# arancormonk/dsd-neo

Hardware: AMD Instinct MI355X
Metric: I/Q Msamples/s end-to-end (demod->FEC->MBE) per GPU; % HBM roofline (higher is better)
Workload: dtype f32

## Files before the change

dsd-neo_amd/csrc/ddn_block.hip:

```cpp

#include <hip/hip_runtime.h>
#include <stdint.h>

#include <stdlib.h>
#include "ddn_device.h"
#include "ddn_nid_dev.h"

using namespace ddn_nid;

__global__ __launch_bounds__(64) void
k_nid_decode(const uint8_t* __restrict__ bits63, const uint8_t* __restrict__ rel63, const int32_t* __restrict__ obs_nac,
             const uint8_t* __restrict__ parity, const uint8_t* __restrict__ parity_rel, int threshold, int n,
             int32_t* __restrict__ out4, int32_t* __restrict__ chase_list, int32_t* __restrict__ chase_count) {
    __shared__ uint8_t ex[128];
    __shared__ uint8_t lg[64];
    __shared__ uint8_t work[(23 + 24 + 24 + 24) * 64];
    if (threadIdx.x == 0) {
        gf_fill(ex, lg);
    }
    __syncthreads();
    const Gf gf = {ex, lg};
    const Work wk = {work + threadIdx.x, work + 23 * 64 + threadIdx.x, work + 47 * 64 + threadIdx.x,
                     work + 71 * 64 + threadIdx.x};
    const int c = blockIdx.x * blockDim.x + threadIdx.x;
// ... 7 lines not shown
    }
    const int par = parity ? (parity[c] ? 1 : 0) : 0;
    const int prel = parity_rel ? parity_rel[c] : 0;
    const int obs = obs_nac ? obs_nac[c] : 0;
    const bool obs_ok = obs > 0 && obs < 0xFFF;

    int failed = 0;
    NidRes hard = nid_codeword(gf, wk, w, par, &failed);
    if (hard.status == 0 && failed && obs_ok && rx_nac(w) != obs) {
        hard = nid_codeword(gf, wk, put_nac(w, obs), par, nullptr);
    }
    NidRes res = hard;
    if (hard.status <= 0 && rel63 && chase_list) {
        chase_list[atomicAdd(chase_count, 1)] = c;
    } else if (hard.status <= 0 && rel63) {
        const uint8_t* rel = rel63 + (size_t)c * 63;
        uint64_t pool = 0;
        uint64_t taken = 0;
        int below = 0;
        for (int i = 0; i < 63; i++) {
            below += rel[i] < threshold;
        }
        for (int k = 0; k < 8; k++) {
            int bi = -1, bv = 256;
            for (int i = 0; i < 63; i++) {
                if (!((taken >> i) & 1) && rel[i] < bv) {
                    bv = rel[i];
                    bi = i;
                }
            }
            pool |= (uint64_t)bi << (8 * k);
            taken |= 1ull << bi;
        }
        int np = below < 8 ? below : 8;
        if (np < 6) {
            np = 6;
        }
        ChaseBest best = {0, {0, 0, 0, 0}, 0, 0};
        chase_from(gf, wk, w, rel, pool, np, par, prel, threshold, &best);
        if (obs_ok && rx_nac(w) != obs) {
            chase_from(gf, wk, put_nac(w, obs), rel, pool, np, par, prel, threshold, &best);
        }
        if (best.found) {
            res = best.dec;
        }
    }
    int32_t* o = out4 + (size_t)c * 4;
    o[0] = res.status;
    o[1] = res.nac;
    o[2] = res.duid;
    o[3] = res.errs;
}

__global__ void
k_hamming_10_6_3(uint8_t* __restrict__ bits10, int n, uint8_t* __restrict__ errs, DdnSel sel) {
    auto one = [&](long c) {
    uint8_t* b = bits10 + (size_t)c * 10;
    int word = 0;
    bool bad = false;
    for (int i = 0; i < 10; i++) {
        bad |= b[i] > 1;
        word = (word << 1) | (b[i] & 1);
    }
    if (bad) {
        errs[c] = 2;
        return;
    }
    const int masks[4] = {0x398, 0x354, 0x2E2, 0x1E1};
    int syn = 0;
    for (int k = 0; k < 4; k++) {
        syn = (syn << 1) | (__popc((unsigned)(word & masks[k])) & 1);
    }
    int e = 0;
    if (syn) {
        const int8_t bad_bit[16] = {-2, 0, 1, 5, 2, -1, -1, 6, 3, -1, -1, 7, 4, 8, 9, -1};
        const int bb = bad_bit[syn];
        if (bb < 0) {
            e = 2;
        } else {
            e = 1;
            if (bb >= 4) {
                word ^= 1 << bb;
            }
            for (int i = 0; i < 6; i++) {
                b[i] = (uint8_t)((word >> (9 - i)) & 1);
            }
        }
    }
    errs[c] = (uint8_t)e;
    };
    ddn_sel_for_each(sel, (long)n, one);
}

__global__ __launch_bounds__(64) void
k_nid_chase(const uint8_t* __restrict__ bits63, const uint8_t* __restrict__ rel63, const int32_t* __restrict__ obs_nac,
            const uint8_t* __restrict__ parity, const uint8_t* __restrict__ parity_rel, int threshold,
            const int32_t* __restrict__ chase_list, const int32_t* __restrict__ chase_count, int32_t* __restrict__ out4) {
    __shared__ uint8_t ex[128];
    __shared__ uint8_t lg[64];
    __shared__ uint8_t work[(23 + 24 + 24 + 24) * 64];
    __shared__ uint8_t masks[96];
    if ((int)blockIdx.x >= *chase_count) {
        return;
    }
    const int lane = threadIdx.x;
    if (lane == 0) {
        gf_fill(ex, lg);
// ... 170 lines not shown
            (void)hipFreeAsync(scratch, st);
        }
        return e;
    }
    hipLaunchKernelGGL(k_nid_chase, dim3((unsigned)n), dim3(64), 0, st, bits63, rel63, obs_nac, parity, parity_rel,
                       threshold, (const int32_t*)list, (const int32_t*)count, out4);
    e = hipGetLastError();
    const hipError_t ef = hipFreeAsync(scratch, st);
    return e != hipSuccess ? e : ef;
}

extern "C" hipError_t
ddn_dev_hamming_10_6_3(uint8_t* bits10, int n, uint8_t* errs, hipStream_t st) {
    if (n <= 0) {
        return hipSuccess;
    }
    const DdnSel sel = ddn_sel_for(24);
    hipLaunchKernelGGL(k_hamming_10_6_3, dim3(ddn_sel_grid(&sel, ((unsigned long)n + DDN_WG - 1) / DDN_WG)), dim3(DDN_WG), 0, st, bits10, n, errs, sel);
    return hipGetLastError();
}

namespace {
__device__ __forceinline__ int
lsd_parity_of(int data) {
    int v = data << 8;
#pragma unroll
    for (int i = 15; i >= 8; i--) {
        if (v & (1 << i)) {
            v ^= 0x139 << (i - 8);
        }
    }
    return v & 0xFF;
}

__device__ __forceinline__ int
lsd_hard(int word) {
    const int data = (word >> 8) & 0xFF, parity = word & 0xFF;
    const int synd = parity ^ lsd_parity_of(data);
    if (synd == 0) {
        return word;
    }
    if ((synd & (synd - 1)) == 0) {
        return word ^ synd;
    }
#pragma unroll
    for (int pos = 0; pos < 8; pos++) {
        if (lsd_parity_of(1 << (7 - pos)) == synd) {
            return word ^ (1 << (15 - pos));
        }
    }
    return -1;
}

__global__ void
k_p25_lsd(uint8_t* __restrict__ bits16, const int16_t* __restrict__ llr16, int n, uint8_t* __restrict__ ok, DdnSel sel) {
    auto one = [&](long i) {
    uint8_t* b = bits16 + (size_t)i * 16;
    int word = 0;
    for (int k = 0; k < 16; k++) {
        word = (word << 1) | (b[k] & 1);
    }
    int fixed = lsd_hard(word);
    if (fixed < 0 && llr16) {
        const int16_t* l = llr16 + (size_t)i * 16;
        int cand[6], rel[6], nc = 0;
        unsigned taken = 0;
        for (int c = 0; c < 6; c++) {
            int bi = -1, br = 1 << 30;
            for (int k = 0; k < 16; k++) {
                const int r = l[k] < 0 ? -(int)l[k] : (int)l[k];
                if (r < 64 && !(taken & (1u << k)) && r < br) {
                    br = r;
                    bi = k;
                }
            }
            if (bi < 0) {
                break;
            }
            taken |= 1u << bi;
            cand[nc] = bi;
            rel[nc] = br;
            nc++;
        }
        int best = -1, best_pen = 999999;
        for (int mask = 1; mask < (1 << nc); mask++) {
            int w = word, pen = 0;
            for (int c = 0; c < nc; c++) {
                if (mask & (1 << c)) {
                    w ^= 1 << (15 - cand[c]);
                    pen += rel[c];
                }
            }
            if (pen >= best_pen) {
                continue;
            }
            const int f = lsd_hard(w);
            if (f >= 0) {
                best = f;
                best_pen = pen;
            }
        }
        fixed = best;
    }
    if (fixed >= 0) {
        for (int k = 0; k < 16; k++) {
            b[k] = (uint8_t)((fixed >> (15 - k)) & 1);
        }
    }
    ok[i] = fixed >= 0 ? 1 : 0;
    };
    ddn_sel_for_each(sel, (long)n, one);
}
}

extern "C" hipError_t
ddn_dev_p25_lsd(uint8_t* bits16, const int16_t* llr16, int n, uint8_t* ok, hipStream_t st) {
    if (n <= 0) {
        return hipSuccess;
    }
    const DdnSel sel = ddn_sel_for(2);
    hipLaunchKernelGGL(k_p25_lsd, dim3(ddn_sel_grid(&sel, ((unsigned long)n + DDN_WG - 1) / DDN_WG)), dim3(DDN_WG), 0, st, bits16, llr16, n, ok, sel);
    return hipGetLastError();
}

namespace {
__global__ void
k_p25_crc16(const uint8_t* __restrict__ bytes, int item_bytes, int n, uint8_t* __restrict__ ok) {
    const int i = blockIdx.x * blockDim.x + threadIdx.x;
    if (i >= n) {
        return;
    }
    const uint8_t* b = bytes + (size_t)i * item_bytes;
    unsigned crc = 0;
    for (int k = 0; k < item_bytes - 2; k++) {
        const unsigned v = b[k];
#pragma unroll
        for (int j = 7; j >= 0; j--) {
            const unsigned bit = (v >> j) & 1u;
            crc = (((crc >> 15) & 1u) ^ bit) ? (((crc << 1) ^ 0x1021u) & 0xFFFFu) : ((crc << 1) & 0xFFFFu);
        }
    }
    crc ^= 0xFFFFu;
    ok[i] = crc == (((unsigned)b[item_bytes - 2] << 8) | b[item_bytes - 1]) ? 1 : 0;
// ... 12 lines not shown
```

dsd-neo_amd/csrc/ddn_mbe.hip:

```cpp

#include <hip/hip_runtime.h>
#include <mutex>
#include <stdint.h>

#include "ddn_device.h"
#include "ddn_mbe.h"
#include "ddn_mbe_dev.h"
#include "ddn_mbe_math.h"

namespace {

__device__ __forceinline__ uint32_t
golay_syndrome(uint32_t w) {
#pragma unroll
    for (int i = 22; i >= 11; i--) {
        if ((w >> i) & 1u) {
            w ^= 0xC75u << (i - 11);
        }
    }
    return w & 0x7FFu;
}

__device__ __forceinline__ void
golay_table_lds(uint32_t* tab, int tid, int nthreads) {
// ... 1 lines not shown
        const int a = idx / 529, b = (idx / 23) % 23, c = idx % 23;
        if (a <= b && b <= c) {
            const uint32_t e = (1u << a) | (1u << b) | (1u << c);
            tab[golay_syndrome(e)] = e;
        }
    }
    if (tid == 0) {
        tab[0] = 0;
    }
}

__device__ uint32_t g_golay_tab[2048];

__global__ __launch_bounds__(256) void
k_golay_tab_init() {
    __shared__ uint32_t tab[2048];
    for (int i = threadIdx.x; i < 2048; i += 256) {
        tab[i] = 0;
    }
    __syncthreads();
    golay_table_lds(tab, threadIdx.x, 256);
    __syncthreads();
    for (int i = threadIdx.x; i < 2048; i += 256) {
        g_golay_tab[i] = tab[i];
    }
}

__device__ __forceinline__ uint32_t
golay_fix(uint32_t w, const uint32_t* tab, int& errs) {
    const uint32_t e = tab[golay_syndrome(w)] & 0x7FF800u;
    errs = __popc(e);
    return w ^ e;
}

__device__ __forceinline__ uint32_t
hamming_fix(uint32_t w, int& errs) {
    const uint32_t m0 = 0x7f08, m1 = 0x78e4, m2 = 0x66d2, m3 = 0x55b1;
    const uint32_t syn = ((__popc(w & m0) & 1) << 3) | ((__popc(w & m1) & 1) << 2) | ((__popc(w & m2) & 1) << 1)
                         | (__popc(w & m3) & 1);
    errs = 0;
    if (syn) {
        errs = 1;
#pragma unroll
        for (int p = 0; p < 15; p++) {
            const uint32_t col = (((m0 >> p) & 1u) << 3) | (((m1 >> p) & 1u) << 2) | (((m2 >> p) & 1u) << 1) | ((m3 >> p) & 1u);
            if (col == syn) {
                w ^= 1u << p;
            }
        }
    }
    return w;
}

#define DDN_MBE_FRAMES_PER_WG 32
template <int CODEC>
__global__ __launch_bounds__(64) void
k_mbe_frame_decode(const uint8_t* __restrict__ frames, const uint8_t* __restrict__ soft, size_t n,
                   uint8_t* __restrict__ bits_out, int32_t* __restrict__ result) {
    constexpr int FB = CODEC == DDN_MBE_IMBE_7200X4400 ? 184 : 96;
    constexpr int OB = CODEC == DDN_MBE_IMBE_7200X4400 ? 88 : 49;
    constexpr int ROWLEN = CODEC == DDN_MBE_IMBE_7200X4400 ? 23 : 24;
    constexpr int FPW = DDN_MBE_FRAMES_PER_WG;
    __shared__ uint8_t stage[FPW * FB];
    __shared__ uint8_t outb[FPW * OB];
    const uint32_t* tab = g_golay_tab;
    const int lane = threadIdx.x;
    const size_t f0 = (size_t)blockIdx.x * FPW;
    const size_t nf = (n - f0) < (size_t)FPW ? (n - f0) : (size_t)FPW;
    const uint8_t* src = frames + f0 * FB;
    for (size_t i = lane; i < nf * FB; i += 64) {
        stage[i] = src[i];
    }
    __syncthreads();
    if ((size_t)lane < nf) {
        const uint8_t* f = stage + lane * FB;
        uint32_t row[8];
        bool bad = false;
        constexpr int NROW = CODEC == DDN_MBE_IMBE_7200X4400 ? 8 : 4;
#pragma unroll
        for (int r = 0; r < NROW; r++) {
            uint32_t w = 0;
            for (int j = 0; j < ROWLEN; j++) {
                const uint32_t v = f[r * ROWLEN + j];
                bad |= v > 1u;
                w |= (v & 1u) << j;
            }
            row[r] = w;
        }
        uint8_t* o = outb + lane * OB;
        int c0 = 0, c4 = 0, total = 0, e = 0;
        unsigned flags = MBE_PROCESS_FLAG_C0_VALID | (soft ? MBE_PROCESS_FLAG_SOFT_INPUT : 0u);
        if (CODEC == DDN_MBE_IMBE_7200X4400) {
            flags |= MBE_PROCESS_FLAG_C4_VALID;
            row[0] = golay_fix(row[0], tab, c0);
            total = c0;
            uint32_t pr = (16u * (row[0] >> 11)) & 0xFFFFu;
#pragma unroll
            for (int r = 1; r < 7; r++) {
                const int len = r < 4 ? 23 : 15;
                uint32_t mask = 0;
                for (int j = len - 1; j >= 0; j--) {
                    pr = (173u * pr + 13849u) & 0xFFFFu;
                    mask |= (pr >> 15) << j;
                }
                row[r] ^= mask;
            }
#pragma unroll
            for (int r = 1; r < 4; r++) {
                row[r] = golay_fix(row[r], tab, e);
                total += e;
            }
#pragma unroll
            for (int r = 4; r < 7; r++) {
                row[r] = hamming_fix(row[r] & 0x7FFFu, e);
                if (r == 4) {
                    c4 = e;
                }
                total += e;
            }
            int k = 0;
#pragma unroll
            for (int r = 0; r < 4; r++) {
                for (int j = 22; j > 10; j--) {
                    o[k++] = (uint8_t)((row[r] >> j) & 1u);
                }
            }
#pragma unroll
            for (int r = 4; r < 7; r++) {
                for (int j = 14; j >= 4; j--) {
                    o[k++] = (uint8_t)((row[r] >> j) & 1u);
                }
            }
            for (int j = 6; j >= 0; j--) {
                o[k++] = (uint8_t)((row[7] >> j) & 1u);
            }
        } else {
            uint32_t w0 = golay_fix(row[0] >> 1, tab, c0);
            row[0] = (w0 << 1) | (row[0] & 1u);
            uint32_t pr = (16u * (w0 >> 11)) & 0xFFFFu;
            uint32_t mask = 0;
            for (int j = 22; j >= 0; j--) {
                pr = (173u * pr + 13849u) & 0xFFFFu;
                mask |= (pr >> 15) << j;
            }
            row[1] = golay_fix((row[1] ^ mask) & 0x7FFFFFu, tab, e);
            total = c0 + e;
            int k = 0;
            for (int j = 23; j > 11; j--) {
                o[k++] = (uint8_t)((row[0] >> j) & 1u);
            }
            for (int j = 22; j > 10; j--) {
                o[k++] = (uint8_t)((row[1] >> j) & 1u);
            }
            for (int j = 10; j >= 0; j--) {
                o[k++] = (uint8_t)((row[2] >> j) & 1u);
            }
            for (int j = 13; j >= 0; j--) {
                o[k++] = (uint8_t)((row[3] >> j) & 1u);
            }
        }
        int32_t* r5 = result + (f0 + lane) * 5;
        if (bad) {
            for (int k = 0; k < OB; k++) {
                o[k] = 0;
            }
            r5[0] = (int32_t)DDN_MBE_RESULT_INVALID;
            r5[1] = r5[2] = r5[3] = r5[4] = 0;
        } else {
            r5[0] = (int32_t)flags;
            r5[1] = c0;
            r5[2] = c4;
            r5[3] = total;
            r5[4] = total - c0;
        }
    }
    __syncthreads();
    uint8_t* dst = bits_out + f0 * OB;
    for (size_t i = lane; i < nf * OB; i += 64) {
        dst[i] = outb[i];
    }
}

struct LaneParms {
    float w0, gamma;
    int L, K, repeat;
    int V;
    float Ml, log2Ml, PHI, PSI;
};

__device__ __forceinline__ LaneParms
lane_init(int l) {
    LaneParms p;
    p.w0 = 0.09378f;
    p.gamma = 0.0f;
    p.L = 30;
    p.K = 10;
    p.repeat = 0;
    p.V = 0;
    p.Ml = 0.0f;
    p.log2Ml = 0.0f;
    p.PHI = 0.0f;
    p.PSI = MBE_PI_F / 2.0f;
    (void)l;
    return p;
}

__device__ __forceinline__ LaneParms
lane_load(const mbe_parms* s, int l) {
    LaneParms p;
    const int i = l <= 56 ? l : 56;
    p.w0 = s->w0;
    p.gamma = s->gamma;
    p.L = s->L;
    p.K = s->K;
    p.repeat = s->repeat;
    p.V = s->Vl[i];
    p.Ml = s->Ml[i];
    p.log2Ml = s->log2Ml[i];
    p.PHI = s->PHIl[i];
    p.PSI = s->PSIl[i];
    return p;
}

__device__ __forceinline__ void
lane_store(mbe_parms* s, const LaneParms& p, int l, int un) {
    if (l == 0) {
        s->w0 = p.w0;
        s->gamma = p.gamma;
        s->L = p.L;
        s->K = p.K;
        s->repeat = p.repeat;
        s->un = un;
    }
    if (l <= 56) {
        s->Vl[l] = p.V;
        s->Ml[l] = p.Ml;
        s->log2Ml[l] = p.log2Ml;
        s->PHIl[l] = p.PHI;
        s->PSIl[l] = p.PSI;
    }
}

__device__ __forceinline__ float
dequant(uint32_t b, int bits, float step) {
    if (bits <= 0) {
        return 0.0f;
    }
    return step * (((float)b - (float)(1u << (bits - 1))) + 0.5f);
}

__device__ __forceinline__ float
idct_term(const float* C, int J, int j) {
    float acc = 0.0f;
    for (int k = 1; k <= J; k++) {
        const float a = (k == 1) ? 1.0f : 2.0f;
        const float ang = (MBE_PI_F * (float)(k - 1) * ((float)j - 0.5f)) / (float)J;
        acc = acc + (a * C[k]) * mbe_cosf(ang);
    }
    return acc;
}

template <int CODEC>
__global__ __launch_bounds__(64) void
k_mbe_params(const uint8_t* __restrict__ bits, const int32_t* __restrict__ res_in, int n_frames,
             const ddn_mbe_tables* __restrict__ T, const float* __restrict__ half_log2, DdnMbeStream* __restrict__ streams,
             int tail_rule, DdnMbeFrameRec* __restrict__ recs, int32_t* __restrict__ res_out) {
    constexpr int NB = CODEC == DDN_MBE_IMBE_7200X4400 ? 88 : 49;
    __shared__ uint32_t fld[64];
    __shared__ float sG[12], sR[12], sC[64], sPl[64], sA[64], sB[64];
    __shared__ float sCb[5][64];
    const int s = blockIdx.x;
    const int l = threadIdx.x;
    DdnMbeStream* st = streams + s;
    LaneParms cur = lane_load(&st->cur, l), prev = lane_load(&st->prev, l), enh = lane_load(&st->enh, l);
    uint32_t frame_no = st->frame_no;
    const uint32_t seed = st->seed;

    for (int f = 0; f < n_frames; f++) {
        const size_t fi = (size_t)s * (size_t)n_frames + (size_t)f;
        const uint8_t* d = bits + fi * NB;
        int32_t r[5] = {0, 0, 0, 0, 0};
        if (res_in) {
#pragma unroll
            for (int k = 0; k < 5; k++) {
                r[k] = res_in[fi * 5 + k];
            }
        }
        unsigned flags = (unsigned)r[0];
        const int errs2 = r[3];
        DdnMbeFrameRec* rec = recs + fi;
        const uint32_t v0 = (l < NB) ? d[l] : 0u, v1 = (l + 64 < NB) ? d[l + 64] : 0u;
        const unsigned long long m0 = __ballot(v0 & 1u), m1 = __ballot(v1 & 1u);
        const bool invalid = __any((v0 > 1u) || (v1 > 1u)) || (flags & DDN_MBE_RESULT_INVALID);
        auto bit = [&](int p) -> uint32_t { return (uint32_t)(((p < 64 ? m0 >> p : m1 >> (p - 64))) & 1ull); };
        bool skip = invalid;
        if (!skip && tail_rule && CODEC == DDN_MBE_IMBE_7200X4400 && errs2 >= 10) {
            uint32_t prefix = 0;
            for (int p = 0; p < 8; p++) {
                prefix = (prefix << 1) | bit(p);
            }
            const int set = __popcll(m0) + __popcll(m1 & 0xFFFFFFull);
            if (prefix == 0xFCu && set <= 24) {
                skip = true;
                flags = 0;
                r[1] = r[2] = r[3] = r[4] = 0;
            }
        }
        if (skip) {
            if (l == 0) {
                rec->flags = DDN_MBE_REC_SILENCE;
                rec->maxl = 0;
                if (res_out) {
                    res_out[fi * 5 + 0] = (int32_t)(invalid ? DDN_MBE_RESULT_INVALID : flags);
                    res_out[fi * 5 + 1] = r[1];
                    res_out[fi * 5 + 2] = r[2];
                    res_out[fi * 5 + 3] = r[3];
                    res_out[fi * 5 + 4] = r[4];
                }
            }
            continue;
        }

        cur.repeat = prev.repeat;
        int bad = 0;
        float Tl = 0.0f;
        float rho = 0.65f, extra = 0.0f;
        int L = 0;
        float unvc = 1.0f;
        if (CODEC == DDN_MBE_IMBE_7200X4400) {
            uint32_t b0 = 0;
            for (int p = 0; p < 6; p++) {
// ... 131 lines not shown
                    sG[l] = T->ambe_prba24[b3][l - 2];
                } else if (l >= 5 && l <= 8) {
                    sG[l] = T->ambe_prba58[b4][l - 5];
                }
                __syncthreads();
                if (l >= 1 && l <= 8) {
                    sR[l] = idct_term(sG, 8, l);
                }
                __syncthreads();
                for (int i = 1; i <= 4; i++) {
                    sCb[i][l] = 0.0f;
                }
                __syncthreads();
                if (l < 24) {
                    const int i = l / 6 + 1, k = l % 6 + 1;
                    const int J = T->ambe_blocks[L][i - 1];
                    float c = 0.0f;
                    if (k == 1) {
                        c = 0.5f * (sR[2 * i - 1] + sR[2 * i]);
                    } else if (k == 2) {
                        c = 0.353553390593274f * (sR[2 * i - 1] - sR[2 * i]);
                    } else if (k <= J) {
                        const float* h = (i == 1) ? T->ambe_hoc5[b5] : ((i == 2) ? T->ambe_hoc6[b6] : ((i == 3) ? T->ambe_hoc7[b7] : T->ambe_hoc8[b8]));
                        c = h[k - 3];
                    }
                    sCb[i][k] = c;
                }
                __syncthreads();
                if (l >= 1 && l <= L) {
                    int first = 1, bi = 1, J = 1;
                    for (int i = 1; i <= 4; i++) {
                        J = T->ambe_blocks[L][i - 1];
                        bi = i;
                        if (l < first + J) {
                            break;
                        }
                        first += J;
                    }
                    Tl = idct_term(sCb[bi], J, l - first + 1);
                }
                sA[l] = Tl;
                __syncthreads();
                float tsum = 0.0f;
                for (int k = 1; k <= L; k++) {
                    tsum = tsum + sA[k];
                }
                extra = (cur.gamma - half_log2[L]) - (tsum / (float)L);
                rho = 0.65f;
                __syncthreads();
            }
        }
        if (bad == 0) {
            const int pL = prev.L;
            const float pl_edge = __shfl(prev.log2Ml, pL <= 56 ? pL : 56);
            const float pl_one = __shfl(prev.log2Ml, 1);
            sPl[l] = (l == 0) ? pl_one : ((l <= pL && l <= 56) ? prev.log2Ml : pl_edge);
            __syncthreads();
            const float ratio = (float)pL / (float)L;
            float sum = 0.0f;
            for (int k = 1; k <= L; k++) {
                const float kl = ratio * (float)k;
                const int ki = (int)kl;
                const float dl = kl - (float)ki;
                sum = sum + (((1.0f - dl) * sPl[ki]) + (dl * sPl[ki + 1]));
            }
            sum = sum * (rho / (float)L);
            if (l >= 1 && l <= L) {
                const float kl = ratio * (float)l;
                const int ki = (int)kl;
                const float dl = kl - (float)ki;
                cur.log2Ml = (((Tl + ((rho * (1.0f - dl)) * sPl[ki])) + ((rho * dl) * sPl[ki + 1])) - sum) + extra;
                const float m = mbe_expf(0.693f * cur.log2Ml);
                cur.Ml = (CODEC == DDN_MBE_AMBE_3600X2450 && !cur.V) ? unvc * m : m;
            }
            __syncthreads();
        }
        bool use_last;
        if (CODEC == DDN_MBE_IMBE_7200X4400) {
            use_last = (bad == 1) || (errs2 > 5);
        } else {
            use_last = (bad == 0) && (errs2 > 3);
        }
        if (use_last) {
            const int rp = cur.repeat;
            cur = prev;
            cur.repeat = rp + 1;
            flags |= MBE_PROCESS_FLAG_REPEAT;
        } else {
            cur.repeat = 0;
        }
        if ((CODEC == DDN_MBE_IMBE_7200X4400 || bad == 0) && cur.repeat <= 3) {
            prev = cur;
            const int cL = cur.L;
            const float cw = mbe_cosf(cur.w0 * (float)l);
            const float m2 = cur.Ml * cur.Ml;
            sA[l] = m2;
            sB[l] = m2 * cw;
            __syncthreads();
            float Rm0 = 0.0f, Rm1 = 0.0f;
            for (int k = 1; k <= cL; k++) {
                Rm0 = Rm0 + sA[k];
                Rm1 = Rm1 + sB[k];
            }
            __syncthreads();
            const float R2m0 = Rm0 * Rm0, R2m1 = Rm1 * Rm1;
            if (l >= 1 && l <= cL && cur.Ml != 0.0f) {
                const float num = (0.96f * MBE_PI_F) * ((R2m0 + R2m1) - (((2.0f * Rm0) * Rm1) * cw));
                const float den = (cur.w0 * Rm0) * (R2m0 - R2m1);
                const float x = num / den;
                float W = 1.0f;
                if (!((8 * l) <= cL || !(x > 0.0f) || !(x < 3.0e38f))) {
                    const float tmp = sqrtf(cur.Ml) * sqrtf(sqrtf(x));
                    W = (tmp > 1.2f) ? 1.2f : ((tmp < 0.5f) ? 0.5f : tmp);
                }
                cur.Ml = cur.Ml * W;
            }
            sA[l] = cur.Ml * cur.Ml;
            __syncthreads();
            float sum2 = 0.0f;
            for (int k = 1; k <= cL; k++) {
                sum2 = sum2 + sA[k];
            }
            __syncthreads();
            const float gam = (sum2 == 0.0f) ? 1.0f : sqrtf(Rm0 / sum2);
            if (l >= 1 && l <= cL) {
                cur.Ml = gam * cur.Ml;
            }
            const int num_uv = __popcll(__ballot(l >= 1 && l <= cL && cur.V == 0));
            const float cw0 = cur.w0, pw0 = enh.w0;
            int maxl;
            if (cL > enh.L) {
                maxl = cL;
                if (l > enh.L && l <= maxl) {
                    enh.Ml = 0.0f;
                    enh.V = 1;
                }
            } else {
                maxl = enh.L;
                if (l > cL && l <= maxl) {
                    cur.Ml = 0.0f;
                    cur.V = 1;
                }
            }
            const uint32_t fbase = mbe_mix(mbe_mix(0x9E3779B9u, seed), frame_no);
            if (l >= 1 && l <= 56) {
                float psi = enh.PSI + ((pw0 + cw0) * ((float)(l * 160) / 2.0f));
                psi = __builtin_fmaf(-__builtin_rintf(psi * 0.159154943091895336f), MBE_TWO_PI_F, psi);
                cur.PSI = psi;
                if (l <= (cL / 4)) {
                    cur.PHI = psi;
                } else {
                    cur.PHI = psi + (((float)num_uv * mbe_rand_phase(mbe_mix(mbe_mix(fbase, (uint32_t)l), 0x100u))) / (float)cL);
                }
            }
            const unsigned long long cvm = __ballot(cur.V != 0), pvm = __ballot(enh.V != 0);
            rec->cMl[l] = cur.Ml;
            rec->pMl[l] = enh.Ml;
            rec->cPHI[l] = cur.PHI;
            rec->pPHI[l] = enh.PHI;
            if (l == 0) {
                rec->cw0 = cw0;
                rec->pw0 = pw0;
                rec->maxl = maxl;
                rec->flags = 0;
                rec->cv_lo = (uint32_t)cvm;
                rec->cv_hi = (uint32_t)(cvm >> 32);
                rec->pv_lo = (uint32_t)pvm;
                rec->pv_hi = (uint32_t)(pvm >> 32);
                rec->fbase = fbase;
            }
            enh = cur;
        } else {
            flags |= MBE_PROCESS_FLAG_MUTE;
            cur = prev = enh = lane_init(l);
            if (l == 0) {
                rec->flags = DDN_MBE_REC_SILENCE;
                rec->maxl = 0;
            }
        }
        frame_no++;
        if (l == 0 && res_out) {
            res_out[fi * 5 + 0] = (int32_t)flags;
            res_out[fi * 5 + 1] = r[1];
            res_out[fi * 5 + 2] = r[2];
            res_out[fi * 5 + 3] = r[3];
            res_out[fi * 5 + 4] = r[4];
        }
    }
    lane_store(&st->cur, cur, l, (int)frame_no);
    lane_store(&st->prev, prev, l, (int)frame_no);
    lane_store(&st->enh, enh, l, (int)frame_no);
    if (l == 0) {
        st->frame_no = frame_no;
    }
}

__device__ __forceinline__ float
unvoiced_mix(float w0, float w0l, int l, int n, uint32_t base, uint32_t tag) {
    float c3 = 0.0f;
#pragma unroll
    for (int i = 0; i < 3; i++) {
        const float rph = mbe_rand_phase(mbe_mix(base, tag + (uint32_t)i));
        c3 = c3 + mbe_cosf(((w0 * (float)n) * (((float)l + ((float)i * MBE_UVSTEP)) - MBE_UVOFFSET)) + rph);
        if (w0l > MBE_UVTHRESHOLD) {
            c3 = c3 + (((w0l - MBE_UVTHRESHOLD) * MBE_UVRAND) * mbe_u01(mbe_mix(mbe_mix(base, tag + 0x40u + (uint32_t)i), (uint32_t)n)));
        }
    }
    return c3;
}

__global__ __launch_bounds__(64) void
k_mbe_synth(const DdnMbeFrameRec* __restrict__ recs, float* __restrict__ pcm) {
    const DdnMbeFrameRec* rec = recs + blockIdx.x;
    float* out = pcm + (size_t)blockIdx.x * 160;
    const int lane = threadIdx.x;
    const int maxl = rec->maxl;
    float acc[3] = {0.0f, 0.0f, 0.0f};
    if (!(rec->flags & DDN_MBE_REC_SILENCE)) {
        const float cw0 = rec->cw0, pw0 = rec->pw0;
        const uint32_t fbase = rec->fbase;
        const unsigned long long cvm = ((unsigned long long)rec->cv_hi << 32) | rec->cv_lo;
        const unsigned long long pvm = ((unsigned long long)rec->pv_hi << 32) | rec->pv_lo;
        const int nA = lane, nB = 56 + lane, nC = 105 + lane;
        const bool inA = lane < 56, inB = lane < 49, inC = lane < 55;
        const float wpA = mbe_ws(nA + 160), wpB = mbe_ws(nB + 160), wcB = mbe_ws(nB), wcC = mbe_ws(nC);
        for (int l = 1; l <= maxl; l++) {
            const float cw0l = cw0 * (float)l, pw0l = pw0 * (float)l;
            const uint32_t base = mbe_mix(fbase, (uint32_t)l);
            const int cv = (int)((cvm >> l) & 1ull), pv = (int)((pvm >> l) & 1ull);
            const float cM = rec->cMl[l], pM = rec->pMl[l], cP = rec->cPHI[l], pP = rec->pPHI[l];
            auto prev_side = [&](int n, float w) {
                if (pv == 1) {
                    return (w * pM) * mbe_cosf((pw0l * (float)n) + pP);
                }
                const float c3 = unvoiced_mix(pw0, pw0l, l, n, base, 0x300u);
                return (((c3 * MBE_UVSINE) * w) * pM) * MBE_QFACTOR;
            };
            auto cur_side = [&](int n, float w) {
                if (cv == 1) {
                    return (w * cM) * mbe_cosf((cw0l * (float)(n - 160)) + cP);
                }
                const float c3 = unvoiced_mix(cw0, cw0l, l, n, base, 0x200u);
                return (((c3 * MBE_UVSINE) * w) * cM) * MBE_QFACTOR;
// ... 132 lines not shown
```

dsd-neo_amd/csrc/ddn_rs.hip:

```cpp

#include <hip/hip_runtime.h>

#include <mutex>
#include <stdint.h>

#include "ddn_device.h"
#include "ddn_tables_isch.h"

namespace {
__device__ __forceinline__ uint32_t
golay_syndrome11(uint32_t cw) {
    cw &= 0x7fffffu;
#pragma unroll
    for (int i = 0; i < 12; i++) {
        cw = (cw & 1u) ? ((cw ^ 0xAE3u) >> 1) : (cw >> 1);
    }
    return cw;
}
}

__global__ void
k_golay_table(uint32_t* __restrict__ tab) {
    const int idx = blockIdx.x * blockDim.x + threadIdx.x;
    if (idx == 0) {
// ... 14 lines not shown
    auto one = [&](long i) {
    uint8_t* d = data + (size_t)i * len;
    const uint8_t* p = parity + (size_t)i * 12;
    uint32_t cw = 0;
    bool valid = true;
    for (int k = 0; k < 12; k++) {
        const uint32_t v = p[k];
        valid &= v <= 1;
        cw |= (v & 1u) << (12 + k);
    }
    for (int k = 0; k < len; k++) {
        const uint32_t v = d[k];
        valid &= v <= 1;
        cw |= (v & 1u) << (12 - len + k);
    }
    int fx = 0, rc = 1;
    if (valid) {
        const uint32_t pbit = cw & 0x800000u;
        uint32_t w23 = cw & 0x7fffffu;
        const uint32_t e = tab[golay_syndrome11(w23)];
        if (e) {
            const int wt = __popc(e);
            bool fits = false;
            uint32_t r = e;
#pragma unroll
            for (int k = 0; k < 23; k++) {
                fits |= (r & 0xFFFu) == 0;
                r = ((r << 1) | (r >> 22)) & 0x7fffffu;
            }
            fx = fits ? wt : wt - 1;
            w23 ^= e;
        }
        cw = w23 | pbit;
        const bool odd = (__popc(cw) & 1) != 0;
        if (!(odd && (cw & 0x3fu) != 0)) {
            rc = 0;
            for (int k = 0; k < len; k++) {
                d[k] = (uint8_t)((cw >> (12 - len + k)) & 1u);
            }
        }
    }
    status[i] = (uint8_t)rc;
    if (fixed) {
        fixed[i] = fx;
    }
    };
    ddn_sel_for_each(sel, (long)n, one);
}

__global__ __launch_bounds__(64) void
k_rs63(uint8_t* __restrict__ data6, const uint8_t* __restrict__ parity6, int n_par, int n_data, int t, int n,
       uint8_t* __restrict__ status, DdnSel sel) {
    __shared__ uint8_t ex[128], lg[64];
    __shared__ uint8_t W[36][64];
    __shared__ uint8_t S[17][64], Cc[18][64], Bb[18][64], Tt[18][64], Om[16][64], Pos[8][64];
    const int lane = threadIdx.x;
    if (lane == 0) {
        int x = 1;
        for (int i = 0; i < 63; i++) {
            ex[i] = (uint8_t)x;
            ex[i + 63] = (uint8_t)x;
            lg[x] = (uint8_t)i;
            x <<= 1;
            if (x & 0x40) {
                x ^= 0x43;
            }
        }
        ex[126] = ex[0];
        ex[127] = ex[1];
        lg[0] = 0;
    }
    __syncthreads();
    auto one = [&](long i) {
    auto gmul = [&](int a, int b) -> int { return (a && b) ? ex[lg[a] + lg[b]] : 0; };
    auto gdiv = [&](int a, int b) -> int { return a ? ex[lg[a] + 63 - lg[b]] : 0; };
    auto gpow = [&](int a, int e) -> int { return a ? ex[(lg[a] + e) % 63] : 0; };
    const int nsym = n_par + n_data, n2 = 2 * t;
    uint8_t* dp = data6 + (size_t)i * n_data * 6;
    const uint8_t* pp = parity6 + (size_t)i * n_par * 6;
    for (int k = 0; k < nsym; k++) {
        const uint8_t* q = (k < n_par) ? (pp + 6 * k) : (dp + 6 * (k - n_par));
        int v = 0;
#pragma unroll
        for (int b = 0; b < 6; b++) {
            v = (v << 1) | (q[b] != 0);
        }
        W[k][lane] = (uint8_t)v;
    }
    int any = 0;
    for (int s = 1; s <= n2; s++) {
        int acc = 0;
        for (int j = 0; j < nsym; j++) {
            acc ^= gpow(W[j][lane], (s * j) % 63);
        }
        S[s][lane] = (uint8_t)acc;
        any |= acc;
    }
    int rc = 0;
    if (any) {
        for (int k = 0; k < 18; k++) {
            Cc[k][lane] = (k == 0);
            Bb[k][lane] = (k == 0);
        }
        int L = 0, m = 1, b = 1;
        for (int it = 0; it < n2; it++) {
            int d = S[it + 1][lane];
            for (int k = 1; k <= L; k++) {
                d ^= gmul(Cc[k][lane], S[it + 1 - k][lane]);
            }
            if (d == 0) {
                m++;
            } else {
                const int f = gdiv(d, b);
                const bool grow = 2 * L <= it;
                for (int k = 0; k < 18; k++) {
                    Tt[k][lane] = Cc[k][lane];
                }
                for (int k = 0; k + m < 18; k++) {
                    Cc[k + m][lane] ^= (uint8_t)gmul(f, Bb[k][lane]);
                }
                if (grow) {
                    L = it + 1 - L;
                    for (int k = 0; k < 18; k++) {
                        Bb[k][lane] = Tt[k][lane];
                    }
                    b = d;
                    m = 1;
                } else {
                    m++;
                }
            }
        }
        int deg = 0;
        for (int k = 17; k >= 0; k--) {
            if (Cc[k][lane]) {
                deg = k;
                break;
            }
        }
        if (L > t || deg != L) {
            rc = 1;
        } else {
            int np = 0;
            for (int p = 0; p < 63; p++) {
                const int xi = (63 - p) % 63;
                int v = 0;
                for (int k = 0; k <= L; k++) {
                    v ^= gpow(Cc[k][lane], (k * xi) % 63);
                }
                if (v == 0) {
                    if (np < 8) {
                        Pos[np][lane] = (uint8_t)p;
                    }
                    np++;
                }
            }
            if (np != L) {
                rc = 1;
            } else {
                for (int k = 0; k < n2; k++) {
                    int v = 0;
                    for (int j = 0; j <= k && j <= L; j++) {
                        v ^= gmul(Cc[j][lane], S[k - j + 1][lane]);
                    }
                    Om[k][lane] = (uint8_t)v;
                }
                int ev[8];
                for (int k = 0; k < 8; k++) {
                    ev[k] = 0;
                }
                for (int e = 0; e < L && rc == 0; e++) {
                    const int p = Pos[e][lane];
                    const int xi = (63 - p) % 63;
                    int num = 0, den = 0;
                    for (int k = 0; k < n2; k++) {
                        num ^= gpow(Om[k][lane], (k * xi) % 63);
                    }
                    for (int k = 1; k <= L; k += 2) {
                        den ^= gpow(Cc[k][lane], ((k - 1) * xi) % 63);
                    }
                    if (den == 0) {
                        rc = 1;
                    } else {
                        const int val = gdiv(num, den);
#pragma unroll
                        for (int k = 0; k < 8; k++) {
                            ev[k] = (k == e) ? val : ev[k];
                        }
                    }
                }
                if (rc == 0) {
#pragma unroll
                    for (int e = 0; e < 8; e++) {
                        if (e < L) {
                            const int p = Pos[e][lane];
                            if (p < nsym) {
                                W[p][lane] ^= (uint8_t)ev[e];
                            }
                        }
                    }
                    for (int k = 0; k < n_data; k++) {
                        const int v = W[n_par + k][lane];
#pragma unroll
                        for (int b = 0; b < 6; b++) {
                            dp[6 * k + b] = (uint8_t)((v >> (5 - b)) & 1);
                        }
                    }
                }
            }
        }
    } else {
        for (int k = 0; k < n_data; k++) {
            const int v = W[n_par + k][lane];
#pragma unroll
            for (int b = 0; b < 6; b++) {
                dp[6 * k + b] = (uint8_t)((v >> (5 - b)) & 1);
            }
        }
    }
    if (rc != 0) {
        for (int k = 0; k < n_data; k++) {
            const int v = W[n_par + k][lane];
#pragma unroll
            for (int b = 0; b < 6; b++) {
                dp[6 * k + b] = (uint8_t)((v >> (5 - b)) & 1);
            }
        }
    }
    status[i] = (uint8_t)rc;
    };
    ddn_sel_for_each(sel, (long)n, one);
}

__global__ __launch_bounds__(64) void
k_rs63_soft(uint8_t* __restrict__ data6, const uint8_t* __restrict__ parity6, const uint8_t* __restrict__ data_rel,
            const uint8_t* __restrict__ parity_rel, int n_par, int n_data, int t, int threshold, int n,
            uint8_t* __restrict__ status) {
    __shared__ uint8_t ex[128], lg[64];
    __shared__ uint8_t W[36][64], S[17][64], G[18][64], M[17][64], Cc[18][64], Bb[18][64], Tt[18][64], Lam[18][64],
        Om[16][64], Loc[16][64], Val[16][64], Er[16][64];
    __shared__ uint16_t Key[36][64];
    const int lane = threadIdx.x;
    if (lane == 0) {
        int x = 1;
        for (int i = 0; i < 63; i++) {
            ex[i] = (uint8_t)x;
            ex[i + 63] = (uint8_t)x;
            lg[x] = (uint8_t)i;
            x <<= 1;
            if (x & 0x40) {
                x ^= 0x43;
            }
        }
        ex[126] = ex[0];
        ex[127] = ex[1];
        lg[0] = 0;
    }
    __syncthreads();
    const int i = blockIdx.x * 64 + lane;
    if (i >= n) {
        return;
    }
    auto gmul = [&](int a, int b) -> int { return (a && b) ? ex[lg[a] + lg[b]] : 0; };
    auto gdiv = [&](int a, int b) -> int { return a ? ex[lg[a] + 63 - lg[b]] : 0; };
    auto gpow = [&](int a, int e) -> int { return a ? ex[(lg[a] + e) % 63] : 0; };
    const int nsym = n_par + n_data, n2 = 2 * t;
    uint8_t* dp = data6 + (size_t)i * n_data * 6;
    const uint8_t* pp = parity6 + (size_t)i * n_par * 6;
    for (int k = 0; k < nsym; k++) {
        const uint8_t* q = (k < n_par) ? (pp + 6 * k) : (dp + 6 * (k - n_par));
        int v = 0;
#pragma unroll
        for (int b = 0; b < 6; b++) {
            v = (v << 1) | (q[b] != 0);
        }
        W[k][lane] = (uint8_t)v;
    }
    int any = 0;
    for (int s = 1; s <= n2; s++) {
        int acc = 0;
// ... 1329 lines not shown
```

Baseline: 25300.

## Bit-pack MBE frame staging, slim RS63 shared memory, and add launch bounds

The MBE frame decoder now packs input bits into 32-bit words in LDS using 8-byte loads and a multiply trick, builds output fields in registers, and writes the output with 4-byte stores. Frames per workgroup rise to 64. RS63 drops the W and Tt shared arrays, computing syndromes incrementally and fusing the Berlekamp-Massey copy with the update. The LSD soft-decision search packs its candidates into one 64-bit key word, two block kernels gain launch bounds, and the MBE synthesis keeps prev/enh history in LDS to relieve register pressure. Together these aim to cut LDS footprint, byte-wise memory traffic and register use, but they add more index arithmetic and extra LDS round trips.

```diff
diff --git a/dsd-neo_amd/csrc/ddn_block.hip b/dsd-neo_amd/csrc/ddn_block.hip
--- a/dsd-neo_amd/csrc/ddn_block.hip
+++ b/dsd-neo_amd/csrc/ddn_block.hip
@@ -83,7 +83,7 @@
     o[3] = res.errs;
 }
 
-__global__ void
+__global__ __launch_bounds__(DDN_WG) void
 k_hamming_10_6_3(uint8_t* __restrict__ bits10, int n, uint8_t* __restrict__ errs, DdnSel sel) {
     auto one = [&](long c) {
     uint8_t* b = bits10 + (size_t)c * 10;
@@ -360,7 +360,7 @@
     return -1;
 }
 
-__global__ void
+__global__ __launch_bounds__(DDN_WG) void
 k_p25_lsd(uint8_t* __restrict__ bits16, const int16_t* __restrict__ llr16, int n, uint8_t* __restrict__ ok, DdnSel sel) {
     auto one = [&](long i) {
     uint8_t* b = bits16 + (size_t)i * 16;
@@ -371,23 +371,22 @@
     int fixed = lsd_hard(word);
     if (fixed < 0 && llr16) {
         const int16_t* l = llr16 + (size_t)i * 16;
-        int cand[6], rel[6], nc = 0;
-        unsigned taken = 0;
+        unsigned long long cands = 0;
+        int nc = 0, prev = -1;
         for (int c = 0; c < 6; c++) {
-            int bi = -1, br = 1 << 30;
+            int bk = 1 << 30;
             for (int k = 0; k < 16; k++) {
                 const int r = l[k] < 0 ? -(int)l[k] : (int)l[k];
-                if (r < 64 && !(taken & (1u << k)) && r < br) {
-                    br = r;
-                    bi = k;
+                const int key = (r << 4) | k;
+                if (r < 64 && key > prev && key < bk) {
+                    bk = key;
                 }
             }
-            if (bi < 0) {
+            if (bk == (1 << 30)) {
                 break;
             }
-            taken |= 1u << bi;
-            cand[nc] = bi;
-            rel[nc] = br;
+            prev = bk;
+            cands |= (unsigned long long)bk << (10 * c);
             nc++;
         }
         int best = -1, best_pen = 999999;
@@ -395,8 +394,9 @@
             int w = word, pen = 0;
             for (int c = 0; c < nc; c++) {
                 if (mask & (1 << c)) {
-                    w ^= 1 << (15 - cand[c]);
-                    pen += rel[c];
+                    const int key = (int)(cands >> (10 * c)) & 0x3FF;
+                    w ^= 1 << (15 - (key & 15));
+                    pen += key >> 4;
                 }
             }
             if (pen >= best_pen) {
diff --git a/dsd-neo_amd/csrc/ddn_mbe.hip b/dsd-neo_amd/csrc/ddn_mbe.hip
--- a/dsd-neo_amd/csrc/ddn_mbe.hip
+++ b/dsd-neo_amd/csrc/ddn_mbe.hip
@@ -77,7 +77,20 @@
     return w;
 }
 
-#define DDN_MBE_FRAMES_PER_WG 32
+__device__ __forceinline__ void
+bits_append_msb(uint64_t& lo, uint64_t& hi, int pos, uint32_t field, int len) {
+    const uint64_t v = (uint64_t)(__brev(field) >> (32 - len));
+    if (pos < 64) {
+        lo |= v << pos;
+        if (pos + len > 64) {
+            hi |= v >> (64 - pos);
+        }
+    } else {
+        hi |= v << (pos - 64);
+    }
+}
+
+#define DDN_MBE_FRAMES_PER_WG 64
 template <int CODEC>
 __global__ __launch_bounds__(64) void
 k_mbe_frame_decode(const uint8_t* __restrict__ frames, const uint8_t* __restrict__ soft, size_t n,
@@ -86,33 +99,46 @@
     constexpr int OB = CODEC == DDN_MBE_IMBE_7200X4400 ? 88 : 49;
     constexpr int ROWLEN = CODEC == DDN_MBE_IMBE_7200X4400 ? 23 : 24;
     constexpr int FPW = DDN_MBE_FRAMES_PER_WG;
-    __shared__ uint8_t stage[FPW * FB];
-    __shared__ uint8_t outb[FPW * OB];
+    constexpr int IW = (FB + 31) / 32, OW = (OB + 31) / 32;
+    __shared__ uint32_t sin[FPW * IW];
+    __shared__ uint32_t sout[FPW * OW];
+    __shared__ uint8_t sbad[FPW];
     const uint32_t* tab = g_golay_tab;
     const int lane = threadIdx.x;
     const size_t f0 = (size_t)blockIdx.x * FPW;
-    const size_t nf = (n - f0) < (size_t)FPW ? (n - f0) : (size_t)FPW;
+    const int nf = (int)((n - f0) < (size_t)FPW ? (n - f0) : (size_t)FPW);
     const uint8_t* src = frames + f0 * FB;
-    for (size_t i = lane; i < nf * FB; i += 64) {
-        stage[i] = src[i];
-    }
+    sbad[lane] = 0;
     __syncthreads();
-    if ((size_t)lane < nf) {
-        const uint8_t* f = stage + lane * FB;
+    for (int i = lane; i < nf * (FB / 8); i += 64) {
+        uint32_t v[2];
+        __builtin_memcpy(v, src + (size_t)i * 8, 8);
+        const uint32_t b8 = (((v[0] & 0x01010101u) * 0x10204080u) >> 28) | ((((v[1] & 0x01010101u) * 0x10204080u) >> 28) << 4);
+        const int fr = i / (FB / 8), k = i - fr * (FB / 8);
+        reinterpret_cast<uint8_t*>(sin)[fr * (IW * 4) + k] = (uint8_t)b8;
+        if ((v[0] | v[1]) & 0xFEFEFEFEu) {
+            sbad[fr] = 1;
+        }
+    }
+    __syncthreads();
+    if (lane < nf) {
+        uint32_t in[IW + 1];
+#pragma unroll
+        for (int k = 0; k < IW; k++) {
+            in[k] = sin[lane * IW + k];
+        }
+        in[IW] = 0;
         uint32_t row[8];
-        bool bad = false;
+        const bool bad = sbad[lane] != 0;
         constexpr int NROW = CODEC == DDN_MBE_IMBE_7200X4400 ? 8 : 4;
 #pragma unroll
         for (int r = 0; r < NROW; r++) {
-            uint32_t w = 0;
-            for (int j = 0; j < ROWLEN; j++) {
-                const uint32_t v = f[r * ROWLEN + j];
-                bad |= v > 1u;
-                w |= (v & 1u) << j;
-            }
-            row[r] = w;
-        }
-        uint8_t* o = outb + lane * OB;
+            constexpr uint32_t rmask = (1u << ROWLEN) - 1u;
+            const int p = r * ROWLEN;
+            const uint64_t two = ((uint64_t)in[p / 32 + 1] << 32) | in[p / 32];
+            row[r] = (uint32_t)(two >> (p % 32)) & rmask;
+        }
+        uint64_t olo = 0, ohi = 0;
         int c0 = 0, c4 = 0, total = 0, e = 0;
         unsigned flags = MBE_PROCESS_FLAG_C0_VALID | (soft ? MBE_PROCESS_FLAG_SOFT_INPUT : 0u);
         if (CODEC == DDN_MBE_IMBE_7200X4400) {
@@ -143,22 +169,15 @@
                 }
                 total += e;
             }
-            int k = 0;
 #pragma unroll
             for (int r = 0; r < 4; r++) {
-                for (int j = 22; j > 10; j--) {
-                    o[k++] = (uint8_t)((row[r] >> j) & 1u);
-                }
+                bits_append_msb(olo, ohi, 12 * r, (row[r] >> 11) & 0xFFFu, 12);
             }
 #pragma unroll
             for (int r = 4; r < 7; r++) {
-                for (int j = 14; j >= 4; j--) {
-                    o[k++] = (uint8_t)((row[r] >> j) & 1u);
-                }
-            }
-            for (int j = 6; j >= 0; j--) {
-                o[k++] = (uint8_t)((row[7] >> j) & 1u);
-            }
+                bits_append_msb(olo, ohi, 48 + 11 * (r - 4), (row[r] >> 4) & 0x7FFu, 11);
+            }
+            bits_append_msb(olo, ohi, 81, row[7] & 0x7Fu, 7);
         } else {
             uint32_t w0 = golay_fix(row[0] >> 1, tab, c0);
             row[0] = (w0 << 1) | (row[0] & 1u);
@@ -170,25 +189,14 @@
             }
             row[1] = golay_fix((row[1] ^ mask) & 0x7FFFFFu, tab, e);
             total = c0 + e;
-            int k = 0;
-            for (int j = 23; j > 11; j--) {
-                o[k++] = (uint8_t)((row[0] >> j) & 1u);
-            }
-            for (int j = 22; j > 10; j--) {
-                o[k++] = (uint8_t)((row[1] >> j) & 1u);
-            }
-            for (int j = 10; j >= 0; j--) {
-                o[k++] = (uint8_t)((row[2] >> j) & 1u);
-            }
-            for (int j = 13; j >= 0; j--) {
-                o[k++] = (uint8_t)((row[3] >> j) & 1u);
-            }
+            bits_append_msb(olo, ohi, 0, (row[0] >> 12) & 0xFFFu, 12);
+            bits_append_msb(olo, ohi, 12, (row[1] >> 11) & 0xFFFu, 12);
+            bits_append_msb(olo, ohi, 24, row[2] & 0x7FFu, 11);
+            bits_append_msb(olo, ohi, 35, row[3] & 0x3FFFu, 14);
         }
         int32_t* r5 = result + (f0 + lane) * 5;
         if (bad) {
-            for (int k = 0; k < OB; k++) {
-                o[k] = 0;
-            }
+            olo = ohi = 0;
             r5[0] = (int32_t)DDN_MBE_RESULT_INVALID;
             r5[1] = r5[2] = r5[3] = r5[4] = 0;
         } else {
@@ -198,11 +206,25 @@
             r5[3] = total;
             r5[4] = total - c0;
         }
+        sout[lane * OW] = (uint32_t)olo;
+        sout[lane * OW + 1] = (uint32_t)(olo >> 32);
+        if (OW > 2) {
+            sout[lane * OW + 2] = (uint32_t)ohi;
+        }
     }
     __syncthreads();
     uint8_t* dst = bits_out + f0 * OB;
-    for (size_t i = lane; i < nf * OB; i += 64) {
-        dst[i] = outb[i];
+    auto out_byte = [&](int i) -> uint32_t {
+        const int fr = i / OB, k = i - fr * OB;
+        return (sout[fr * OW + (k >> 5)] >> (k & 31)) & 1u;
+    };
+    const int total = nf * OB;
+    for (int i = lane; i < total / 4; i += 64) {
+        const uint32_t w = out_byte(4 * i) | (out_byte(4 * i + 1) << 8) | (out_byte(4 * i + 2) << 16) | (out_byte(4 * i + 3) << 24);
+        __builtin_memcpy(dst + (size_t)i * 4, &w, 4);
+    }
+    if (lane < (total & 3)) {
+        dst[(total & ~3) + lane] = (uint8_t)out_byte((total & ~3) + lane);
     }
 }
 
@@ -266,6 +288,25 @@
     }
 }
 
+#define DDN_MBE_HIST_ROWS 5
+__device__ __forceinline__ void
+hist_put(uint32_t* h, int l, const LaneParms& p) {
+    h[0 * 64 + l] = (uint32_t)p.V;
+    h[1 * 64 + l] = __float_as_uint(p.Ml);
+    h[2 * 64 + l] = __float_as_uint(p.log2Ml);
+    h[3 * 64 + l] = __float_as_uint(p.PHI);
+    h[4 * 64 + l] = __float_as_uint(p.PSI);
+}
+
+__device__ __forceinline__ void
+hist_get(const uint32_t* h, int l, LaneParms& p) {
+    p.V = (int)h[0 * 64 + l];
+    p.Ml = __uint_as_float(h[1 * 64 + l]);
+    p.log2Ml = __uint_as_float(h[2 * 64 + l]);
+    p.PHI = __uint_as_float(h[3 * 64 + l]);
+    p.PSI = __uint_as_float(h[4 * 64 + l]);
+}
+
 __device__ __forceinline__ float
 dequant(uint32_t b, int bits, float step) {
     if (bits <= 0) {
@@ -294,14 +335,18 @@
     __shared__ uint32_t fld[64];
     __shared__ float sG[12], sR[12], sC[64], sPl[64], sA[64], sB[64];
     __shared__ float sCb[5][64];
+    __shared__ uint32_t hPrev[DDN_MBE_HIST_ROWS * 64], hEnh[DDN_MBE_HIST_ROWS * 64];
     const int s = blockIdx.x;
-    const int l = threadIdx.x;
+    int l = threadIdx.x;
     DdnMbeStream* st = streams + s;
     LaneParms cur = lane_load(&st->cur, l), prev = lane_load(&st->prev, l), enh = lane_load(&st->enh, l);
+    hist_put(hPrev, l, prev);
+    hist_put(hEnh, l, enh);
     uint32_t frame_no = st->frame_no;
     const uint32_t seed = st->seed;
 
     for (int f = 0; f < n_frames; f++) {
+        asm volatile("" : "+v"(l));
         const size_t fi = (size_t)s * (size_t)n_frames + (size_t)f;
         const uint8_t* d = bits + fi * NB;
         int32_t r[5] = {0, 0, 0, 0, 0};
@@ -539,9 +584,10 @@
         }
         if (bad == 0) {
             const int pL = prev.L;
-            const float pl_edge = __shfl(prev.log2Ml, pL <= 56 ? pL : 56);
-            const float pl_one = __shfl(prev.log2Ml, 1);
-            sPl[l] = (l == 0) ? pl_one : ((l <= pL && l <= 56) ? prev.log2Ml : pl_edge);
+            const float pl_own = __uint_as_float(hPrev[2 * 64 + l]);
+            const float pl_edge = __shfl(pl_own, pL <= 56 ? pL : 56);
+            const float pl_one = __shfl(pl_own, 1);
+            sPl[l] = (l == 0) ? pl_one : ((l <= pL && l <= 56) ? pl_own : pl_edge);
             __syncthreads();
             const float ratio = (float)pL / (float)L;
             float sum = 0.0f;
@@ -571,6 +617,7 @@
         if (use_last) {
             const int rp = cur.repeat;
             cur = prev;
+            hist_get(hPrev, l, cur);
             cur.repeat = rp + 1;
             flags |= MBE_PROCESS_FLAG_REPEAT;
         } else {
@@ -578,6 +625,7 @@
         }
         if ((CODEC == DDN_MBE_IMBE_7200X4400 || bad == 0) && cur.repeat <= 3) {
             prev = cur;
+            hist_put(hPrev, l, cur);
             const int cL = cur.L;
             const float cw = mbe_cosf(cur.w0 * (float)l);
             const float m2 = cur.Ml * cur.Ml;
@@ -615,6 +663,7 @@
             }
             const int num_uv = __popcll(__ballot(l >= 1 && l <= cL && cur.V == 0));
             const float cw0 = cur.w0, pw0 = enh.w0;
+            hist_get(hEnh, l, enh);
             int maxl;
             if (cL > enh.L) {
                 maxl = cL;
@@ -657,9 +706,12 @@
                 rec->fbase = fbase;
             }
             enh = cur;
+            hist_put(hEnh, l, cur);
         } else {
             flags |= MBE_PROCESS_FLAG_MUTE;
             cur = prev = enh = lane_init(l);
+            hist_put(hPrev, l, cur);
+            hist_put(hEnh, l, cur);
             if (l == 0) {
                 rec->flags = DDN_MBE_REC_SILENCE;
                 rec->maxl = 0;
@@ -675,7 +727,9 @@
         }
     }
     lane_store(&st->cur, cur, l, (int)frame_no);
+    hist_get(hPrev, l, prev);
     lane_store(&st->prev, prev, l, (int)frame_no);
+    hist_get(hEnh, l, enh);
     lane_store(&st->enh, enh, l, (int)frame_no);
     if (l == 0) {
         st->frame_no = frame_no;
diff --git a/dsd-neo_amd/csrc/ddn_rs.hip b/dsd-neo_amd/csrc/ddn_rs.hip
--- a/dsd-neo_amd/csrc/ddn_rs.hip
+++ b/dsd-neo_amd/csrc/ddn_rs.hip
@@ -90,8 +90,7 @@
 k_rs63(uint8_t* __restrict__ data6, const uint8_t* __restrict__ parity6, int n_par, int n_data, int t, int n,
        uint8_t* __restrict__ status, DdnSel sel) {
     __shared__ uint8_t ex[128], lg[64];
-    __shared__ uint8_t W[36][64];
-    __shared__ uint8_t S[17][64], Cc[18][64], Bb[18][64], Tt[18][64], Om[16][64], Pos[8][64];
+    __shared__ uint8_t S[17][64], Cc[18][64], Bb[18][64], Om[16][64], Pos[8][64];
     const int lane = threadIdx.x;
     if (lane == 0) {
         int x = 1;
@@ -116,23 +115,41 @@
     const int nsym = n_par + n_data, n2 = 2 * t;
     uint8_t* dp = data6 + (size_t)i * n_data * 6;
     const uint8_t* pp = parity6 + (size_t)i * n_par * 6;
-    for (int k = 0; k < nsym; k++) {
-        const uint8_t* q = (k < n_par) ? (pp + 6 * k) : (dp + 6 * (k - n_par));
+    auto symbol = [&](const uint8_t* q) -> int {
         int v = 0;
 #pragma unroll
         for (int b = 0; b < 6; b++) {
             v = (v << 1) | (q[b] != 0);
         }
-        W[k][lane] = (uint8_t)v;
+        return v;
+    };
+    auto rewrite_data = [&]() {
+        for (int k = 0; k < n_data; k++) {
+            const int v = symbol(dp + 6 * k);
+#pragma unroll
+            for (int b = 0; b < 6; b++) {
+                dp[6 * k + b] = (uint8_t)((v >> (5 - b)) & 1);
+            }
+        }
+    };
+    for (int s = 1; s <= n2; s++) {
+        S[s][lane] = 0;
+    }
+    for (int j = 0; j < nsym; j++) {
+        const int v = symbol((j < n_par) ? (pp + 6 * j) : (dp + 6 * (j - n_par)));
+        if (v) {
+            const int lv = lg[v];
+            int e = 0;
+            for (int s = 1; s <= n2; s++) {
+                e += j;
+                e = e >= 63 ? e - 63 : e;
+                S[s][lane] ^= ex[lv + e];
+            }
+        }
     }
     int any = 0;
     for (int s = 1; s <= n2; s++) {
-        int acc = 0;
-        for (int j = 0; j < nsym; j++) {
-            acc ^= gpow(W[j][lane], (s * j) % 63);
-        }
-        S[s][lane] = (uint8_t)acc;
-        any |= acc;
+        any |= S[s][lane];
     }
     int rc = 0;
     if (any) {
@@ -151,20 +168,21 @@
             } else {
                 const int f = gdiv(d, b);
                 const bool grow = 2 * L <= it;
-                for (int k = 0; k < 18; k++) {
-                    Tt[k][lane] = Cc[k][lane];
-                }
-                for (int k = 0; k + m < 18; k++) {
-                    Cc[k + m][lane] ^= (uint8_t)gmul(f, Bb[k][lane]);
-                }
                 if (grow) {
+                    for (int k = 17; k >= 0; k--) {
+                        const uint8_t c = Cc[k][lane];
+                        if (k >= m) {
+                            Cc[k][lane] = c ^ (uint8_t)gmul(f, Bb[k - m][lane]);
+                        }
+                        Bb[k][lane] = c;
+                    }
                     L = it + 1 - L;
-                    for (int k = 0; k < 18; k++) {
-                        Bb[k][lane] = Tt[k][lane];
-                    }
                     b = d;
                     m = 1;
                 } else {
+                    for (int k = 0; k + m < 18; k++) {
+                        Cc[k + m][lane] ^= (uint8_t)gmul(f, Bb[k][lane]);
+                    }
                     m++;
                 }
             }
@@ -228,42 +246,28 @@
                     }
                 }
                 if (rc == 0) {
+                    rewrite_data();
 #pragma unroll
                     for (int e = 0; e < 8; e++) {
                         if (e < L) {
                             const int p = Pos[e][lane];
-                            if (p < nsym) {
-                                W[p][lane] ^= (uint8_t)ev[e];
+                            if (p >= n_par && p < nsym) {
+                                uint8_t* q = dp + 6 * (p - n_par);
+#pragma unroll
+                                for (int b = 0; b < 6; b++) {
+                                    q[b] ^= (uint8_t)((ev[e] >> (5 - b)) & 1);
+                                }
                             }
                         }
                     }
-                    for (int k = 0; k < n_data; k++) {
-                        const int v = W[n_par + k][lane];
-#pragma unroll
-                        for (int b = 0; b < 6; b++) {
-                            dp[6 * k + b] = (uint8_t)((v >> (5 - b)) & 1);
-                        }
-                    }
                 }
             }
         }
     } else {
-        for (int k = 0; k < n_data; k++) {
-            const int v = W[n_par + k][lane];
-#pragma unroll
-            for (int b = 0; b < 6; b++) {
-                dp[6 * k + b] = (uint8_t)((v >> (5 - b)) & 1);
-            }
-        }
+        rewrite_data();
     }
     if (rc != 0) {
-        for (int k = 0; k < n_data; k++) {
-            const int v = W[n_par + k][lane];
-#pragma unroll
-            for (int b = 0; b < 6; b++) {
-                dp[6 * k + b] = (uint8_t)((v >> (5 - b)) & 1);
-            }
-        }
+        rewrite_data();
     }
     status[i] = (uint8_t)rc;
     };
```

After: 25170. Within noise of the previous version (-0.5%).
